# GaetanBenoitDev/metaMDBG

Measured on AMD Instinct MI355X. Metric: Gbp/s through minimizer+k-min-mer step; bit-exact k-min-mer table vs ref, higher is better.
Workload: dtype u64

## Files before the change

include/mdbg_hip.h:

```cpp
#ifndef MDBG_HIP_H
#define MDBG_HIP_H

#include <stddef.h>
#include <stdint.h>

#ifdef __cplusplus
extern "C" {
#endif

#define MDBG_OK        0
#define MDBG_EINVAL   -1
#define MDBG_ENODEV   -2
#define MDBG_ENOMEM   -3
#define MDBG_EHIP     -4
#define MDBG_ERANGE   -5
#define MDBG_EPEER    -6

typedef struct mdbg_ctx mdbg_ctx;
typedef struct mdbg_reads mdbg_reads;
typedef struct mdbg_minimizers mdbg_minimizers;
typedef struct mdbg_table mdbg_table;

int  mdbg_create(int device, mdbg_ctx **ctx);
void mdbg_destroy(mdbg_ctx *ctx);
// ... 76 lines not shown
                              mdbg_table **out);
int  mdbg_prev_from_records(mdbg_ctx *ctx, const uint8_t *records20, uint64_t n_records, mdbg_table **out);
int  mdbg_prev_overlay_unitigs(mdbg_ctx *ctx, mdbg_table *prev, const mdbg_minimizers *unitigs,
                               const uint32_t *abundance, uint32_t k_prev);
int  mdbg_kminmer_count_refined(mdbg_ctx *ctx, const mdbg_minimizers *reads, const mdbg_minimizers *unitigs,
                                uint32_t k, const mdbg_table *prev, mdbg_table **out);
int  mdbg_kminmer_index(mdbg_ctx *ctx, const mdbg_minimizers *reads, const mdbg_minimizers *unitigs,
                        uint32_t k, const mdbg_table *prev, mdbg_table **out);

int  mdbg_small_contigs(mdbg_ctx *ctx, const mdbg_minimizers *unitigs, uint32_t k, uint32_t k_prev, const mdbg_table *prev,
                        uint8_t *flags);

int  mdbg_table_info(const mdbg_table *t, uint32_t *k, uint64_t *n_records, uint64_t *n_solid, int *has_vectors);
int  mdbg_table_to_host(mdbg_ctx *ctx, const mdbg_table *t, uint8_t *records20, uint32_t *vectors);
int  mdbg_table_to_host_range(mdbg_ctx *ctx, const mdbg_table *t, uint64_t first, uint64_t count, uint8_t *records20, uint32_t *vectors);
int  mdbg_table_stats(const mdbg_table *t, uint64_t stats[4]);
int  mdbg_first_pass_info(const mdbg_ctx *ctx, uint64_t info[8]);
int  mdbg_first_pass_form(const mdbg_ctx *ctx, uint64_t form[4]);
int  mdbg_first_pass_slot_fall_backs(const mdbg_ctx *ctx, uint64_t *n);
const char *mdbg_step_kernel_name(uint32_t index);
int  mdbg_kernel_attributes(mdbg_ctx *ctx, const char *kernel, uint64_t attr[8]);
int  mdbg_scan_info(const mdbg_ctx *ctx, uint64_t info[8]);
int  mdbg_scan_confirm_info(const mdbg_ctx *ctx, uint64_t info[4]);
int  mdbg_table_checksum(mdbg_ctx *ctx, const mdbg_table *t, uint64_t sums[4]);
int  mdbg_table_lookup(mdbg_ctx *ctx, const mdbg_table *t, const uint64_t *hash_lo, const uint64_t *hash_hi,
                       uint64_t n, uint32_t *abundance);
int  mdbg_edge_index(mdbg_ctx *ctx, const mdbg_table *nodes, mdbg_table **edges, uint64_t *checksum);
int  mdbg_table_keys_to_host(mdbg_ctx *ctx, const mdbg_table *t, uint64_t *keys_lo_hi);
int  mdbg_unitig_edge_index(mdbg_ctx *ctx, const mdbg_minimizers *unitigs, uint32_t k, mdbg_table **edges, uint64_t *checksum);
void mdbg_table_free(mdbg_table *t);

typedef struct mdbg_spans mdbg_spans;
int  mdbg_kminmer_spans(mdbg_ctx *ctx, const mdbg_reads *reads, const mdbg_minimizers *mins,
                        uint32_t minimizer_size, int32_t hpc, uint32_t k, mdbg_spans **out);
int  mdbg_spans_info(const mdbg_spans *s, uint32_t *n_reads, uint64_t *n_minimizers, uint64_t *n_windows, uint32_t *k);
int  mdbg_spans_to_host(mdbg_ctx *ctx, const mdbg_spans *s, uint64_t *window_offsets,
                        uint32_t *min_start, uint32_t *min_end,
                        uint64_t *hash_lo, uint64_t *hash_hi, uint8_t *reversed,
                        uint32_t *pos_start, uint32_t *pos_end, uint32_t *seq_length_start, uint32_t *seq_length_end);
int  mdbg_spans_device_ptrs(const mdbg_spans *s, const uint64_t **d_window_offsets, const uint64_t **d_hash_lo, const uint64_t **d_hash_hi,
                            const uint32_t **d_pos_start, const uint32_t **d_pos_end);
void mdbg_spans_free(mdbg_spans *s);

typedef struct { uint64_t window; uint32_t part; uint32_t reserved; } mdbg_seq_request;
typedef struct { uint32_t read, start, length, reversed; } mdbg_seq_range;
enum { MDBG_SEQ_ENTIRE = 0, MDBG_SEQ_LEFT = 1, MDBG_SEQ_RIGHT = 2 };
// ... 85 lines not shown
```

metamdbg_amd/capi.py:

```python
from __future__ import annotations

import ctypes as C
import os

import numpy as np

_HERE = os.path.dirname(os.path.abspath(__file__))
LIB_PATH = os.environ.get("MDBG_LIB") or os.path.join(_HERE, "libmdbg_hip.so")

MDBG_READ_LOW_COMPLEXITY = 1
MDBG_READ_LOW_QUALITY = 2
RECORDS_PLAIN, RECORDS_INIT = 0, 1
SEQ_ENTIRE, SEQ_LEFT, SEQ_RIGHT = 0, 1, 2
SEQ_BITSET, SEQ_ASCII = 0, 1
SEQ_REQUEST = np.dtype([("window", "<u8"), ("part", "<u4"), ("reserved", "<u4")])
SEQ_RANGE = np.dtype([("read", "<u4"), ("start", "<u4"), ("length", "<u4"), ("reversed", "<u4")])


class MdbgError(RuntimeError):
    def __init__(self, code: int, msg: str):
        super().__init__(f"libmdbg_hip error {code}: {msg}")
        self.code = code


# ... 42 lines not shown
    "mdbg_minimizers_device_ptrs": (C.c_int, [_P, C.POINTER(_P), C.POINTER(_P)]),
    "mdbg_minimizers_free": (None, [_P]),
    "mdbg_minimizers_concat": (C.c_int, [_P, C.POINTER(_P), C.c_uint32, C.POINTER(_P)]),
    "mdbg_apply_density_threshold": (C.c_int, [_P, _P, C.c_float, C.POINTER(_P)]),
    "mdbg_purge_palindromes": (C.c_int, [_P, _P, C.c_uint32, C.c_uint32, C.POINTER(_P)]),
    "mdbg_repetitive_minimizers": (C.c_int, [_P, _P, _P, _u32p]),
    "mdbg_census_create": (C.c_int, [_P, C.POINTER(_P)]),
    "mdbg_census_add": (C.c_int, [_P, _P, _P]),
    "mdbg_census_top": (C.c_int, [_P, _P, _P, _u32p]),
    "mdbg_census_free": (None, [_P]),
    "mdbg_kminmer_count_first": (C.c_int, [_P, _P, C.c_uint32, C.c_uint32, C.POINTER(_P)]),
    "mdbg_prev_from_records": (C.c_int, [_P, _P, C.c_uint64, C.POINTER(_P)]),
    "mdbg_prev_overlay_unitigs": (C.c_int, [_P, _P, _P, _P, C.c_uint32]),
    "mdbg_kminmer_count_refined": (C.c_int, [_P, _P, _P, C.c_uint32, _P, C.POINTER(_P)]),
    "mdbg_kminmer_index": (C.c_int, [_P, _P, _P, C.c_uint32, _P, C.POINTER(_P)]),
    "mdbg_table_info": (C.c_int, [_P, _u32p, _u64p, _u64p, C.POINTER(C.c_int)]),
    "mdbg_table_to_host": (C.c_int, [_P, _P, _P, _P]),
    "mdbg_table_to_host_range": (C.c_int, [_P, _P, C.c_uint64, C.c_uint64, _P, _P]),
    "mdbg_table_checksum": (C.c_int, [_P, _P, _u64p]),
    "mdbg_table_stats": (C.c_int, [_P, _u64p]),
    "mdbg_first_pass_info": (C.c_int, [_P, _u64p]),
    "mdbg_scan_info": (C.c_int, [_P, _u64p]),
    "mdbg_scan_confirm_info": (C.c_int, [_P, _u64p]),
    "mdbg_first_pass_form": (C.c_int, [_P, _u64p]),
    "mdbg_first_pass_slot_fall_backs": (C.c_int, [_P, _u64p]),
    "mdbg_step_kernel_name": (C.c_char_p, [C.c_uint32]),
    "mdbg_kernel_attributes": (C.c_int, [_P, C.c_char_p, _u64p]),
    "mdbg_stream_spin": (C.c_int, [_P, C.c_uint32]),
    "mdbg_minimizers_slice": (C.c_int, [_P, _P, C.c_uint32, C.c_uint32, C.POINTER(C.c_void_p)]),
    "mdbg_shard_exchange_local": (C.c_int, [_P, C.POINTER(C.c_void_p), C.c_uint32, C.POINTER(C.c_void_p), _u64p, C.POINTER(C.c_void_p)]),
    "mdbg_device_clock_khz": (C.c_int, [_P, C.POINTER(C.c_int)]),
    "mdbg_table_lookup": (C.c_int, [_P, _P, _P, _P, C.c_uint64, _P]),
    "mdbg_edge_index": (C.c_int, [_P, _P, C.POINTER(_P), _u64p]),
    "mdbg_unitig_edge_index": (C.c_int, [_P, _P, C.c_uint32, C.POINTER(_P), _u64p]),
    "mdbg_small_contigs": (C.c_int, [_P, _P, C.c_uint32, C.c_uint32, _P, _P]),
    "mdbg_table_keys_to_host": (C.c_int, [_P, _P, _P]),
    "mdbg_table_free": (None, [_P]),
    "mdbg_kminmer_spans": (C.c_int, [_P, _P, _P, C.c_uint32, C.c_int32, C.c_uint32, C.POINTER(_P)]),
    "mdbg_spans_info": (C.c_int, [_P, _u32p, _u64p, _u64p, _u32p]),
    "mdbg_spans_to_host": (C.c_int, [_P, _P, _P, _P, _P, _P, _P, _P, _P, _P, _P, _P]),
    "mdbg_spans_device_ptrs": (C.c_int, [_P, C.POINTER(_P), C.POINTER(_P), C.POINTER(_P), C.POINTER(_P), C.POINTER(_P)]),
    "mdbg_spans_free": (None, [_P]),
    "mdbg_spans_extract": (C.c_int, [_P, _P, _P, _P, C.c_uint64, C.c_int, C.POINTER(_P)]),
    "mdbg_reads_extract_ranges": (C.c_int, [_P, _P, _P, C.c_uint64, C.c_int, C.POINTER(_P)]),
    "mdbg_sequences_info": (C.c_int, [_P, _u64p, _u64p, _u64p, C.POINTER(C.c_int)]),
    "mdbg_sequences_to_host": (C.c_int, [_P, _P, _P, _P, _P]),
# ... 124 lines not shown
            names.append(name.decode())
            i += 1
        return names

    def kernel_attributes(self, kernel: str) -> dict:
        a = (C.c_uint64 * 8)()
        self.check(lib().mdbg_kernel_attributes(self.h, kernel.encode(), a))
        names = ("registers", "static_lds", "max_threads", "threads", "role", "scratch")
        return {k: int(v) for k, v in zip(names, a)}

    def scan_info(self) -> dict:
        a = (C.c_uint64 * 8)()
        self.check(lib().mdbg_scan_info(self.h, a))
        names = ("prefiltered_launches", "block_launches", "bitmaps_built", "bitmap_bits_set", "bitmap_log2_bits", "prefilter_waves",
                 "last_prefiltered", "reads_segmented")
        return {k: int(v) for k, v in zip(names, a)}

    def scan_confirm_info(self) -> dict:
        a = (C.c_uint64 * 4)()
        self.check(lib().mdbg_scan_confirm_info(self.h, a))
        names = ("tables_built", "table_buckets", "table_overflowed", "last_by_table")
        return {k: int(v) for k, v in zip(names, a)}

    def timing(self, on: bool) -> None:
        self.check(lib().mdbg_timing_enable(self.h, int(on)))

    def timing_reset(self) -> None:
        self.check(lib().mdbg_timing_reset(self.h))

    def timing_get(self, kernel: str) -> tuple[float, int]:
        ms, n = C.c_double(), C.c_uint64()
        self.check(lib().mdbg_timing_get(self.h, kernel.encode(), C.byref(ms), C.byref(n)))
        return ms.value, n.value

    def reads_from_ascii(self, seqs: list[bytes], quals: list[bytes] | None = None) -> "Reads":
        offs = np.zeros(len(seqs) + 1, dtype=np.uint64)
        np.cumsum([len(s) for s in seqs], out=offs[1:])
        bases = b"".join(seqs)
        q = b"".join(quals) if quals is not None else None
        h = C.c_void_p()
        self.check(lib().mdbg_reads_from_ascii(self.h, bases, q, _ptr(offs), len(seqs), C.byref(h)))
        return Reads(self, h)

    def reads_from_packed(self, words: np.ndarray, word_off: np.ndarray, lens: np.ndarray, quals: list[bytes] | None = None) -> "Reads":
        words = np.ascontiguousarray(words, dtype=np.uint64)
        word_off = np.ascontiguousarray(word_off, dtype=np.uint64)
# ... 639 lines not shown
```

metamdbg_amd/csrc/common.hpp:

```cpp
#pragma once
#include <ctime>
#include <cstdio>
#include <cstdlib>

#include <hip/hip_runtime.h>

#include <cstdarg>
#include <cstdint>
#include <cstdio>
#include <cstring>
#include <map>
#include <memory>
#include <mutex>
#include <new>
#include <stdexcept>
#include <string>
#include <unordered_map>
#include <utility>
#include <vector>

#include "../../include/mdbg_hip.h"
#include "segments_dev.hpp"

namespace mdbg {
// ... 104 lines not shown
    unsigned table_blocks_per_cu = 1024;
    unsigned scan_reads_per_wave = 0;
    uint32_t scan_wave_priority = 0;
    int test_exchange_fail_phase = 0;
    bool test_corrupt_replies = false;
    uint32_t scan_cand_slack = 0;
    uint32_t scan_guard_slack = 0;
    uint32_t scan_prefilter = 1;
    uint32_t scan_prefilter_log2_bits = 0;
    uint32_t *prefilter_bits = nullptr;
    bool prefilter_valid = false;
    uint64_t prefilter_threshold = 0;
    uint32_t prefilter_log2 = 0, prefilter_set = 0;
    uint32_t scan_confirm_table = 0;
    uint32_t scan_confirm_table_log2_buckets = 0;
    uint32_t *confirm_table = nullptr;
    bool confirm_valid = false;
    uint64_t confirm_threshold = 0;
    uint32_t confirm_log2 = 0;
    uint64_t scan_confirm_info[4] = {0};
    uint32_t scan_segments = 1;
    uint32_t scan_segment_bases = mdbg::SEG_DEFAULT_BASES;
    uint64_t scan_info[8] = {0};
    double key_ratio_hint[4] = {0.0625, 0.0625, 0.0625, 0.0625};
    bool key_ratio_known[4] = {false, false, false, false};
    int first_pass_mode = 0;
    uint64_t part_auto_min = 1ull << 17;
    uint32_t part_bits = 0;
    uint32_t part_lds_slots = 0;
    uint64_t part_max_records = 0;
    uint32_t part_tile = 0;
    uint32_t part_threads = 0;
    uint64_t part_form[4] = {0};
    uint64_t part_fell_back = 0;
    uint32_t part_slot_list = 1;
    uint32_t scan_lds_pad = 0;
    uint32_t scan_lds_reserve = 0;
    size_t lds_per_cu = 0;
    uint32_t index_table_form = 1;
    uint32_t refined_form = 1;
    uint32_t scan_quality_beside = 1;
    uint32_t keep_index_table = 1;
    double index_last_miss_fraction = -1.0;
    uint32_t index_tuning = INDEX_TUNING_DEFAULT;
    uint64_t part_info[8] = {0};
    std::shared_ptr<mdbg::DevPool> pool;
// ... 185 lines not shown
```

metamdbg_amd/csrc/context.hip:

```cpp
#include "common.hpp"

#include <algorithm>
#include <cstdlib>

namespace mdbg {

thread_local std::string g_last_error;

int set_error(mdbg_ctx *ctx, int code, const char *fmt, ...) {
    char buf[1024];
    va_list ap;
    va_start(ap, fmt);
    vsnprintf(buf, sizeof(buf), fmt, ap);
    va_end(ap);
    if (ctx) ctx->err = buf; else g_last_error = buf;
    return code;
}

static void fold_timers(mdbg_ctx *ctx) {
    if (ctx->launches.empty()) return;
    (void)hipStreamSynchronize(ctx->stream);
    if (ctx->side_stream) (void)hipStreamSynchronize(ctx->side_stream);
    for (auto &t : ctx->launches) {
        float ms = 0;
// ... 20 lines not shown
    if (e != hipSuccess || count == 0)
        return set_error(nullptr, MDBG_ENODEV, "mdbg_create: no HIP device (%s); this library has no CPU path",
                         e != hipSuccess ? hipGetErrorString(e) : "device count is 0");
    if (device < 0 || device >= count)
        return set_error(nullptr, MDBG_EINVAL, "mdbg_create: device %d out of range (%d devices)", device, count);
    hipDeviceProp_t prop;
    if ((e = hipGetDeviceProperties(&prop, device)) != hipSuccess)
        return set_error(nullptr, MDBG_EHIP, "hipGetDeviceProperties: %s", hipGetErrorString(e));
    if (strncmp(prop.gcnArchName, "gfx950", 6) != 0)
        return set_error(nullptr, MDBG_ENODEV, "mdbg_create: device %d is %s; kernels are built for gfx950 only",
                         device, prop.gcnArchName);
    if ((e = hipSetDevice(device)) != hipSuccess)
        return set_error(nullptr, MDBG_EHIP, "hipSetDevice: %s", hipGetErrorString(e));
    mdbg_ctx *ctx = new mdbg_ctx();
    ctx->device = device;
    ctx->arch = prop.gcnArchName;
    ctx->n_cu = prop.multiProcessorCount;
    if (const char *e = getenv("MDBG_TABLE_BLOCKS_PER_CU")) if (atoi(e) > 0) ctx->table_blocks_per_cu = (unsigned)atoi(e);
    if (const char *e = getenv("MDBG_SCAN_WAVE_PRIORITY")) ctx->scan_wave_priority = (uint32_t)std::max(0, std::min(3, atoi(e)));
    if (const char *e = getenv("MDBG_SCAN_READS_PER_WAVE")) if (atoi(e) > 0) ctx->scan_reads_per_wave = (unsigned)atoi(e);
    if (const char *e = getenv("MDBG_SCAN_LDS_RESERVE")) ctx->scan_lds_reserve = (uint32_t)std::max(0, std::min(131072, atoi(e)));
    if (const char *e = getenv("MDBG_SCAN_PREFILTER")) ctx->scan_prefilter = atoi(e) != 0;
    if (const char *e = getenv("MDBG_SCAN_CONFIRM_TABLE")) ctx->scan_confirm_table = atoi(e) != 0;
    if (const char *e = getenv("MDBG_SCAN_SEGMENTS")) ctx->scan_segments = atoi(e) == 0 ? 0u : (atoi(e) == 2 ? 2u : 1u);
    if (const char *e = getenv("MDBG_SCAN_LDS_PAD")) ctx->scan_lds_pad = (uint32_t)std::max(0, std::min(32768, atoi(e)));
    if (const char *e = getenv("MDBG_PARTITION_TILE")) ctx->part_tile = atoi(e) == 2048 ? 2048u : 0u;
    if (const char *e = getenv("MDBG_PARTITION_THREADS")) ctx->part_threads = atoi(e) == 256 ? 256u : (atoi(e) == 512 ? 512u : 0u);
    if (const char *e = getenv("MDBG_PARTITION_SLOT_LIST")) ctx->part_slot_list = atoi(e) != 0;
    if (const char *e = getenv("MDBG_FIRST_PASS_MODE")) ctx->first_pass_mode = std::max(0, std::min(2, atoi(e)));
    ctx->hbm_bytes = prop.totalGlobalMem;
    ctx->lds_per_cu = prop.maxSharedMemoryPerMultiProcessor;
    ctx->clock_khz = prop.clockRate;
    if ((e = hipStreamCreateWithFlags(&ctx->stream, hipStreamNonBlocking)) != hipSuccess ||
        (e = hipStreamCreateWithFlags(&ctx->side_stream, hipStreamNonBlocking)) != hipSuccess) {
        if (ctx->stream) (void)hipStreamDestroy(ctx->stream);
        delete ctx;
        return set_error(nullptr, MDBG_EHIP, "hipStreamCreate: %s", hipGetErrorString(e));
    }
    ctx->pool = std::make_shared<DevPool>();
    ctx->pool->device = device;
    if (ctx->hbm_bytes) ctx->pool->cache_limit = std::max<size_t>(ctx->pool->cache_limit, (size_t)((double)ctx->hbm_bytes * 0.55));
    *out = ctx;
    return MDBG_OK;
} MDBG_API_CATCH((mdbg_ctx *)nullptr)

extern "C" void mdbg_destroy(mdbg_ctx *ctx) {
    if (!ctx) return;
    (void)hipSetDevice(ctx->device);
    fold_timers(ctx);
    (void)hipStreamSynchronize(ctx->stream);
    if (ctx->pool) ctx->pool->close();
    if (ctx->scan_stream) { (void)hipStreamSynchronize(ctx->scan_stream); (void)hipStreamDestroy(ctx->scan_stream); }
    if (ctx->upload_stream) { (void)hipStreamSynchronize(ctx->upload_stream); (void)hipStreamDestroy(ctx->upload_stream); }
    if (ctx->side_stream) { (void)hipStreamSynchronize(ctx->side_stream); (void)hipStreamDestroy(ctx->side_stream); }
    if (ctx->pinned) (void)hipHostFree(ctx->pinned);
    if (ctx->prefilter_bits) { std::lock_guard<std::mutex> g(hip_mem_mutex()); (void)hipFree(ctx->prefilter_bits); }
    if (ctx->confirm_table) { std::lock_guard<std::mutex> g(hip_mem_mutex()); (void)hipFree(ctx->confirm_table); }
    if (ctx->stream) (void)hipStreamDestroy(ctx->stream);
    delete ctx;
}

extern "C" const char *mdbg_last_error(const mdbg_ctx *ctx) {
    return ctx ? ctx->err.c_str() : g_last_error.c_str();
}

extern "C" int mdbg_synchronize(mdbg_ctx *ctx) try {
    if (!ctx) return MDBG_EINVAL;
    MDBG_HIP_CHECK(ctx, hipStreamSynchronize(ctx->stream));
    return MDBG_OK;
} MDBG_API_CATCH(ctx)

__global__ void spin_kernel(long long ticks) {
    const long long t0 = wall_clock64();
    while (wall_clock64() - t0 < ticks) __builtin_amdgcn_s_sleep(8);
}

extern "C" int mdbg_stream_spin(mdbg_ctx *ctx, uint32_t microseconds) try {
    if (!ctx) return MDBG_EINVAL;
    MDBG_HIP_CHECK(ctx, hipSetDevice(ctx->device));
    int khz = 0;
// ... 34 lines not shown
extern "C" int mdbg_set_option(mdbg_ctx *ctx, const char *name, int64_t value) {
    if (!ctx || !name) return set_error(ctx, MDBG_EINVAL, "mdbg_set_option: null argument");
    const std::string n(name);
    if (n == "pool_cache_percent") {
        const int64_t pc = value > 0 ? std::min<int64_t>(value, 95) : 55;
        std::lock_guard<std::mutex> g(ctx->pool->mu);
        ctx->pool->cache_limit = std::max<size_t>((size_t)96 << 30, (size_t)((double)ctx->hbm_bytes * (double)pc / 100.0));
        return MDBG_OK;
    }
    if (n == "pool_trim") {
        MDBG_HIP_CHECK(ctx, hipSetDevice(ctx->device));
        MDBG_HIP_CHECK(ctx, hipStreamSynchronize(ctx->stream));
        ctx->pool->trim();
        return MDBG_OK;
    }
    if (n == "table_cu_count") return set_table_cu_count(ctx, value > 0 ? (unsigned)std::min<int64_t>(value, 4096) : 0u);
    if (n == "table_grid_blocks") { ctx->table_grid_blocks = value > 0 ? (unsigned)std::min<int64_t>(value, 1 << 20) : 0u; return MDBG_OK; }
    if (n == "table_blocks_per_cu") { ctx->table_blocks_per_cu = value > 0 ? (unsigned)std::min<int64_t>(value, 1024) : 1024u; return MDBG_OK; }
    if (n == "scan_wave_priority") { ctx->scan_wave_priority = (uint32_t)std::max<int64_t>(0, std::min<int64_t>(3, value)); return MDBG_OK; }
    if (n == "scan_candidate_slack") { ctx->scan_cand_slack = value > 0 ? (uint32_t)std::min<int64_t>(value, 1 << 24) : 0u; return MDBG_OK; }
    if (n == "scan_guard_slack") { ctx->scan_guard_slack = value > 0 ? (uint32_t)std::min<int64_t>(value, 0xFFFFFFFFll - 68) : 0u; return MDBG_OK; }
    if (n == "scan_prefilter") { ctx->scan_prefilter = value != 0; return MDBG_OK; }
    if (n == "scan_confirm_table") { ctx->scan_confirm_table = value != 0; return MDBG_OK; }
    if (n == "scan_confirm_table_log2_buckets") {
        if (value != 0 && (value < 10 || value > 16)) return set_error(ctx, MDBG_EINVAL, "scan_confirm_table_log2_buckets: 0 (the kernel's own) or 10 .. 16");
        ctx->scan_confirm_table_log2_buckets = (uint32_t)value; return MDBG_OK;
    }
    if (n == "scan_segments") {
        if (value > 2) return set_error(ctx, MDBG_EINVAL, "scan_segments: 0 (never), 1 (automatic, the default; negative too) or 2 (every eligible read)");
        ctx->scan_segments = value < 0 ? 1u : (uint32_t)value; return MDBG_OK;
    }
    if (n == "scan_segment_bases") {
        if (value > 0 && (value % 2048 != 0 || value > (1 << 30))) return set_error(ctx, MDBG_EINVAL, "scan_segment_bases: a multiple of 2048 (<= 0: the default, 16384)");
        ctx->scan_segment_bases = value <= 0 ? SEG_DEFAULT_BASES : (uint32_t)value; return MDBG_OK;
    }
    if (n == "scan_prefilter_log2_bits") {
        if (value != 0 && (value < 10 || value > 19)) return set_error(ctx, MDBG_EINVAL, "scan_prefilter_log2_bits: 0 (the kernel's own) or 10 .. 19");
        ctx->scan_prefilter_log2_bits = (uint32_t)value; return MDBG_OK;
    }
    if (n == "scan_reads_per_wave") { ctx->scan_reads_per_wave = value > 0 ? (unsigned)std::min<int64_t>(value, 1 << 20) : 0u; return MDBG_OK; }
    if (n == "first_pass_mode") { ctx->first_pass_mode = (int)std::max<int64_t>(0, std::min<int64_t>(2, value)); return MDBG_OK; }
    if (n == "partition_auto_min") { ctx->part_auto_min = value > 0 ? (uint64_t)value : (1ull << 17); return MDBG_OK; }
    if (n == "partition_bits") { ctx->part_bits = (uint32_t)std::max<int64_t>(0, std::min<int64_t>(24, value)); return MDBG_OK; }
    if (n == "partition_lds_slots") {
        if (value != 0 && value != 256 && value != 1024 && value != 2048) return set_error(ctx, MDBG_EINVAL, "partition_lds_slots: 0, 256, 1024 or 2048");
        ctx->part_lds_slots = (uint32_t)value; return MDBG_OK;
// ... 72 lines not shown
```

metamdbg_amd/csrc/partition.hip:

```cpp
#include "common.hpp"
#include "kminmer_dev.hpp"
#include "partition_plan.hpp"

#include <algorithm>
#include <cmath>
#include <vector>

namespace mdbg {

#ifndef MDBG_PART_NT
#define MDBG_PART_NT 512
#endif
#ifndef MDBG_PART_E
#define MDBG_PART_E 8
#endif
constexpr uint32_t PART_NT = MDBG_PART_NT;
constexpr uint32_t PART_E = MDBG_PART_E;
constexpr uint32_t PART_TILE = PART_NT * PART_E;
constexpr uint32_t PART_MAXW = 256;
constexpr uint32_t PART_NT_SMALL = 256;
constexpr uint32_t PART_E_SMALL = 4;
constexpr uint32_t PART_TILE_SMALL = PART_NT_SMALL * PART_E_SMALL;
static_assert(PART_NT_SMALL >= PART_MAXW && PART_NT >= PART_MAXW, "the scatter scans a tile's histogram with one thread per way");
constexpr uint32_t PART_MAX_K = 32;
// ... 565 lines not shown
    for (uint64_t i = tid; i < n; i += BC_NT) {
        const uint32_t row = in.rep[s0 + i];
        const uint32_t s = lds_find<C>(t, in.lo[s0 + i], in.hi[s0 + i]);
        reply[row] = (uint64_t)t.cnt[s] | (t.rep[s] == row ? (1ull << 63) : 0ull);
    }
}

struct RecBufs {
    DevBuf<unsigned long long> lo, hi;
    DevBuf<uint32_t> rep;
    uint64_t cap = 0;
    int ensure(mdbg_ctx *ctx, uint64_t n) {
        if (n <= cap) return MDBG_OK;
        MDBG_TRY(lo.alloc(ctx, n)); MDBG_TRY(hi.alloc(ctx, n)); MDBG_TRY(rep.alloc(ctx, n));
        cap = n;
        return MDBG_OK;
    }
    RecView view() { return RecView{lo.p, hi.p, rep.p}; }
};

struct SplitForm { uint32_t threads, tile; };

static SplitForm split_form(const mdbg_ctx *ctx) {
    if (ctx->part_threads == PART_NT_SMALL) return SplitForm{PART_NT_SMALL, PART_TILE_SMALL};
    return SplitForm{PART_NT, ctx->part_tile == 2048 ? PART_TILE / 2 : PART_TILE};
}

static void launch_split_hist(mdbg_ctx *ctx, bool from_mins, SplitForm f, unsigned grid, const SplitArgs &a, uint32_t *hist) {
    if (f.threads == PART_NT_SMALL && PART_NT_SMALL != PART_NT) {
        if (from_mins) hipLaunchKernelGGL((split_hist_kernel<true, PART_NT_SMALL>), dim3(grid), dim3(PART_NT_SMALL), 0, ctx->stream, a, hist);
        else hipLaunchKernelGGL((split_hist_kernel<false, PART_NT_SMALL>), dim3(grid), dim3(PART_NT_SMALL), 0, ctx->stream, a, hist);
    } else {
        if (from_mins) hipLaunchKernelGGL((split_hist_kernel<true, PART_NT>), dim3(grid), dim3(PART_NT), 0, ctx->stream, a, hist);
        else hipLaunchKernelGGL((split_hist_kernel<false, PART_NT>), dim3(grid), dim3(PART_NT), 0, ctx->stream, a, hist);
    }
    ctx->part_form[0] = f.threads; ctx->part_form[1] = f.tile;
}

static void launch_split_scatter(mdbg_ctx *ctx, bool from_mins, SplitForm f, unsigned grid, const SplitArgs &a, const uint64_t *place, RecView out) {
    if (f.tile == PART_TILE_SMALL && f.threads == PART_NT_SMALL) {
        if (from_mins) hipLaunchKernelGGL((split_scatter_kernel<true, PART_E_SMALL, PART_NT_SMALL>), dim3(grid), dim3(PART_NT_SMALL), 0, ctx->stream, a, place, out);
        else hipLaunchKernelGGL((split_scatter_kernel<false, PART_E_SMALL, PART_NT_SMALL>), dim3(grid), dim3(PART_NT_SMALL), 0, ctx->stream, a, place, out);
    } else if (f.tile != PART_TILE) {
        if (from_mins) hipLaunchKernelGGL((split_scatter_kernel<true, PART_E / 2, PART_NT>), dim3(grid), dim3(PART_NT), 0, ctx->stream, a, place, out);
        else hipLaunchKernelGGL((split_scatter_kernel<false, PART_E / 2, PART_NT>), dim3(grid), dim3(PART_NT), 0, ctx->stream, a, place, out);
    } else {
        if (from_mins) hipLaunchKernelGGL((split_scatter_kernel<true, PART_E, PART_NT>), dim3(grid), dim3(PART_NT), 0, ctx->stream, a, place, out);
// ... 550 lines not shown
```

metamdbg_amd/csrc/scan.hip:

```cpp
#include "common.hpp"
#include "complexity_dev.hpp"
#include "murmur.hpp"
#include "objects.hpp"
#include "prefilter.hpp"
#include "scan_plan.hpp"
#include "segments_dev.hpp"

#include <fcntl.h>
#include <sys/file.h>
#include <sys/stat.h>
#include <unistd.h>

#include <algorithm>
#include <cerrno>
#include <cmath>
#include <cstdlib>
#include <memory>
#include <mutex>
#include <string>
#include <thread>
#include <type_traits>

namespace mdbg {

// ... 31 lines not shown
    uint8_t *out_mqual;
    int inline_minq;
    uint32_t *out_count;
    uint8_t *out_flags;
    unsigned long long *cursor;
    uint32_t n_regions;
    uint64_t out_capacity;
    uint64_t *out_begin;
    uint32_t *over_list, *suspect_list;
    uint32_t *list_counters;
    const uint8_t *skip;
    uint32_t cand_slack;
    uint32_t guard_slack;
    uint32_t wave_priority;
    const uint32_t *pf_bits;
    uint32_t pf_shift;
    uint32_t pf_chunk;
    const uint4 *pf_table;
    uint32_t pf_table_shift;
    uint32_t pf_len_split;
    const SegView *views;
    unsigned long long *view_cx;
    uint32_t seg_tiles;
};

__device__ __forceinline__ uint64_t compress_pairs(uint64_t x, uint64_t d) {
    uint64_t xm = x & (d | (d << 1));
    uint32_t xl = (uint32_t)xm, xh = (uint32_t)(xm >> 32);
    uint32_t dl = (uint32_t)d, dh = (uint32_t)(d >> 32);
    uint32_t lo = 0, hi = 0;
    unsigned n = 0;
#pragma unroll
    for (int i = 0; i < 16; i++) {
        lo |= ((xl >> (2 * i)) & 3u) << n;
        n += (dl >> (2 * i) & 1u) << 1;
    }
    const unsigned nlo = n;
    n = 0;
#pragma unroll
    for (int i = 0; i < 16; i++) {
        hi |= ((xh >> (2 * i)) & 3u) << n;
        n += (dh >> (2 * i) & 1u) << 1;
    }
    return (uint64_t)lo | ((uint64_t)hi << nlo);
}

// ... 631 lines not shown
    uint16_t *hist_o = lds_hist_o + ((QUAL && HPC) ? wv * HIST_TILES * 64 : 0);
    uint32_t *hist_c = lds_hist_c[(QUAL && HPC) ? wv : 0];
    const unsigned K = a.K;
    const uint32_t kmask = (K >= 16) ? 0xFFFFFFFFu : ((1u << (2 * K)) - 1u);
    const uint32_t comp_mask = 0xAAAAAAAAu & kmask;
    const unsigned top_shift = 2u * K - 2u;
    const uint64_t threshold = a.threshold;
    const uint64_t cand_limit64 = (threshold >> 32) + 3ull + (uint64_t)a.cand_slack;
    const uint32_t cand_limit = cand_limit64 > 0xFFFFFFFFull ? 0xFFFFFFFFu : (uint32_t)cand_limit64;
    const uint64_t guard_limit64 = 68ull + (uint64_t)a.guard_slack;
    const uint32_t guard_limit = guard_limit64 > 0xFFFFFFFFull ? 0xFFFFFFFFu : (uint32_t)guard_limit64;
    const bool unguarded = HPC && K == 15u && a.guard_slack == 0u;

    const uint32_t wave_global = blockIdx.x * Geo::WAVES + wv;
    const uint32_t n_waves = gridDim.x * Geo::WAVES;
    uint16_t *pf_list = PF ? pf_list_all + wv * PF_LIST_CAP : nullptr;
    uint32_t *pf_surv = PF ? pf_surv_all + wv * 64u : nullptr;
    const uint32_t pf_shift = a.pf_shift;
    const uint4 *const pf_table = PF ? a.pf_table : nullptr;
    const uint32_t pf_table_shift = a.pf_table_shift;
    constexpr uint32_t NO_READ = 0xFFFFFFFFu;
    const uint64_t chunk0 = (uint64_t)blockIdx.x * a.pf_chunk;
    const uint32_t chunk_n = PF ? (chunk0 >= a.n_reads ? 0u : (uint32_t)(a.n_reads - chunk0 < a.pf_chunk ? a.n_reads - chunk0 : a.pf_chunk)) : 0u;
    auto take_read = [&]() -> uint32_t {
        uint32_t k = 0;
        if (lane == 0) k = atomicAdd(pf_next, 1u);
        k = (uint32_t)__builtin_amdgcn_readfirstlane((int)k);
        return k < chunk_n ? (uint32_t)chunk0 + k : NO_READ;
    };
    for (uint32_t r = PF ? take_read() : wave_global; PF ? r != NO_READ : r < a.n_reads; r = PF ? take_read() : r + n_waves) {
        if constexpr (PF && !SEG) { if (a.pf_len_split && a.len[r] >= a.pf_len_split) continue; }
        if (!SEG && a.skip && a.skip[r]) {
            if (a.cursor && lane == 0) { a.out_begin[r] = 0; a.out_count[r] = 0; a.out_flags[r] = 0; }
            continue;
        }
        SegView view{};
        if constexpr (SEG) {
            view = a.views[r];
            if (view.flags & SEG_DEAD) {
                if (lane == 0) { a.out_begin[r] = 0; a.out_count[r] = 0; a.out_flags[r] = 0; a.view_cx[r] = 0ull; }
                continue;
            }
        }
        const uint32_t rd = SEG ? view.read : r;
        const bool seg_inner = SEG && !(view.flags & SEG_FIRST);
        const uint32_t L = SEG ? view.raw_len : a.len[r];
        const uint64_t w_base = a.word_off[rd] + (SEG ? (uint64_t)view.tile0 * TILE_WORDS : 0ull);
// ... 481 lines not shown
            materialise();
            release_ring(((fill + 15u) & ~15u) + 16u);
        }

        if (APPROX && !PF) {
            const uint32_t n_staged = outgrown ? n_staged_at_outgrowth : nout;
            for (uint32_t i = lane; i < ((n_staged + 63u) & ~63u); i += 64) {
                const uint64_t fb = __ballot(i < n_staged && !(kmer_hash32(stage[i].x) < threshold));
                if (fb) { n_false += (uint32_t)__popcll(fb); lost = true; }
            }
        }
        if (((QUAL && HPC) || (APPROX && !PF)) && __ballot(lost) != 0ull) outgrown = true;
        uint8_t flags = 0;
        if constexpr (SEG) {
            const uint64_t cx_view = a.apply_filters ? cx_total + wave_sum_u32(cx_acc) : 0ull;
            if (lane == 0) a.view_cx[r] = cx_view;
        } else if (a.apply_filters && L >= 66) {
            if (complexity_suspect(cx_total + wave_sum_u32(cx_acc), cx_nW)) flags |= READ_SUSPECT;
        }
        if (bump) {
            uint64_t start = 0;
            if (!outgrown && nout) {
                uint32_t lo = 0, hi = 0;
                const uint32_t region = wave_global & (a.n_regions - 1u);
                if (lane == 0) { const unsigned long long s0 = atomicAdd(a.cursor + region, (unsigned long long)nout); lo = (uint32_t)s0; hi = (uint32_t)(s0 >> 32); }
                start = ((uint64_t)(uint32_t)__builtin_amdgcn_readfirstlane((int)hi) << 32) | (uint32_t)__builtin_amdgcn_readfirstlane((int)lo);
                const bool fits = start + nout <= a.out_capacity;
                start += (uint64_t)region * a.out_capacity;
                if (fits) {
                    for (uint32_t i = lane; i < nout; i += 64) {
                        const uint2 e = stage[i];
                        a.out_min[start + i] = e.x; a.out_pos[start + i] = e.y >> 1; a.out_dir[start + i] = (uint8_t)(e.y & 1u);
                        if (QUAL) a.out_mqual[start + i] = stage_q[i];
                    }
                }
            }
            if (lane == 0) {
                a.out_begin[r] = start;
                a.out_count[r] = nout - n_false;
                a.out_flags[r] = flags;
                if (outgrown) a.over_list[atomicAdd(&a.list_counters[0], 1u)] = r;
                if (flags & READ_SUSPECT) a.suspect_list[atomicAdd(&a.list_counters[1], 1u)] = r;
            }
        } else {
            const uint32_t ns = nout - flushed;
            for (uint32_t i = lane; i < ns; i += 64) {
                const uint32_t idx = flushed + i;
// ... 503 lines not shown
        if (!(fast && ctx->scan_stream)) return MDBG_OK;
        MDBG_HIP_CHECK(ctx, hipEventCreateWithFlags(&ordered, hipEventDisableTiming));
        hipError_t e = hipEventRecord(ordered, ctx->stream);
        if (e == hipSuccess) e = hipStreamWaitEvent(ctx->scan_stream, ordered, 0);
        if (e != hipSuccess) { (void)hipEventDestroy(ordered); return set_error(ctx, MDBG_EHIP, "scan stream hand-over: %s", hipGetErrorString(e)); }
        on = ctx->scan_stream;
        return MDBG_OK;
    }
    int give_back(mdbg_ctx *ctx) {
        if (!ordered) return MDBG_OK;
        hipError_t e = hipEventRecord(ordered, on);
        if (e == hipSuccess) e = hipStreamWaitEvent(ctx->stream, ordered, 0);
        (void)hipEventDestroy(ordered);
        if (e != hipSuccess) return set_error(ctx, MDBG_EHIP, "scan stream hand-back: %s", hipGetErrorString(e));
        return MDBG_OK;
    }
};

static unsigned four_wave_lds_pad(const mdbg_ctx *ctx, ScanKernel fk) {
    const bool by_reserve = !ctx->scan_lds_pad && ctx->scan_lds_reserve;
    return scan_lds_padding(ctx->scan_lds_pad, ctx->scan_lds_reserve, ctx->lds_per_cu, by_reserve ? kernel_static_lds(reinterpret_cast<const void *>(fk)) : 0);
}

static int launch_scan(mdbg_ctx *ctx, ScanArgs &a, bool hpc, bool has_q, bool has_n, uint32_t n_items, uint32_t pf_len_limit = 0, bool pf_split = false,
                       uint64_t batch_bases = 0, bool seg = false) {
    a.n_reads = n_items;
    const ScanSwitches &sw = scan_switches();
    const bool fast = (!has_q || a.cursor) && !has_n && !a.subset && !sw.no_fast;
    const bool approx = fast && a.cursor && sw.approx_allowed && candidate_test_usable(a.threshold, a.cand_slack);
    if (seg && !approx) return set_error(ctx, MDBG_EINVAL, "scan: views are scanned by the candidate-hash kernels only");
    unsigned pf_waves = 0;
    MDBG_TRY(choose_prefilter(ctx, a, approx, hpc, has_q, pf_len_limit, &pf_waves));
    pf_split = pf_split && pf_waves;
    DevBuf<uint8_t> d_split;
    if (pf_split) {
        MDBG_TRY(split_long_reads(ctx, a, n_items, pf_len_limit, batch_bases, d_split, &pf_split));
        if (!pf_split) pf_waves = 0;
    }
    ScanStreamLoan loan;
    MDBG_TRY(loan.take(ctx, fast));
    if (fast) ctx->scan_info[6] = pf_waves ? 1 : 0;
    if (fast) ctx->scan_confirm_info[3] = 0;
    {
        LaunchTimer timer(ctx, "scan", loan.on);
        const uint8_t *const batch_skip = a.skip;
        if (pf_split) a.skip = d_split.p;
        if (fast && (!pf_waves || pf_split)) {
            ctx->scan_info[1]++;
            const ScanKernel fk = select_fast_kernel(hpc, has_q, approx, 0, seg);
            hipLaunchKernelGGL(fk, dim3(scan_blocks(n_items, FAST_WAVES, ctx->scan_reads_per_wave)), dim3(FAST_BLOCK), four_wave_lds_pad(ctx, fk), loan.on, a);
        } else if (!fast) {
            hipLaunchKernelGGL(select_general_kernel(hpc, has_q, has_n), dim3(scan_blocks(n_items, SCAN_WAVES, ctx->scan_reads_per_wave)), dim3(SCAN_BLOCK), 0, ctx->stream, a);
        }
        a.skip = batch_skip;
        if (pf_waves) {
            a.pf_bits = ctx->prefilter_bits;
            a.pf_shift = 32u - ctx->prefilter_log2;
            const bool by_table = ctx->scan_confirm_table && ctx->confirm_valid && ctx->confirm_threshold == a.threshold;
            a.pf_table = by_table ? reinterpret_cast<const uint4 *>(ctx->confirm_table) : nullptr;
            a.pf_table_shift = by_table ? 32u - ctx->confirm_log2 : 0u;
            ctx->scan_confirm_info[3] = by_table ? 1 : 0;
            const PrefilterGrid grid = prefilter_grid(n_items, pf_waves, ctx->scan_reads_per_wave, ctx->n_cu);
            a.pf_chunk = grid.chunk;
            a.pf_len_split = pf_split ? pf_len_limit : 0u;
            hipLaunchKernelGGL(select_fast_kernel(true, false, true, pf_waves, seg), dim3(grid.blocks), dim3(64u * pf_waves), 0, loan.on, a);
            ctx->scan_info[0]++; ctx->scan_info[5] = pf_waves;
        }
    }
    MDBG_TRY(loan.give_back(ctx));
    MDBG_HIP_CHECK(ctx, hipGetLastError());
    return MDBG_OK;
}

struct SegPlan : SegTotals {
    DevBuf<uint32_t> tiles_per_read, views_per_read, tile_runs, tile_excl;
    DevBuf<uint64_t> tile_off, view_off;
    DevBuf<SegView> views;
    DevBuf<uint8_t> skip, read_cut;
    DevBuf<unsigned long long> totals;
};

static int seg_prepass(mdbg_ctx *ctx, const mdbg_reads *reads, const uint8_t *masked, uint32_t G, uint32_t K, bool hpc, SegPlan &sp) {
    const uint32_t n = reads->n_reads;
    const uint64_t max_tiles = reads->n_bases / SEG_TILE_BASES + n, max_views = reads->n_bases / G + n;
    MDBG_TRY(sp.tiles_per_read.alloc(ctx, n)); MDBG_TRY(sp.views_per_read.alloc(ctx, n));
    MDBG_TRY(sp.tile_off.alloc(ctx, (size_t)n + 1)); MDBG_TRY(sp.view_off.alloc(ctx, (size_t)n + 1));
    MDBG_TRY(sp.tile_runs.alloc(ctx, hpc ? max_tiles : 1)); MDBG_TRY(sp.tile_excl.alloc(ctx, hpc ? max_tiles : 1));
    MDBG_TRY(sp.views.alloc(ctx, max_views)); MDBG_TRY(sp.skip.alloc(ctx, n)); MDBG_TRY(sp.read_cut.alloc(ctx, n)); MDBG_TRY(sp.totals.alloc(ctx, 8));
// ... 455 lines not shown
    e = hipMemcpyAsync(m->d_len.p, reads->d_len.p, (size_t)n * 4, hipMemcpyDeviceToDevice, ctx->stream);
    if (e != hipSuccess) return set_error(ctx, MDBG_EHIP, "len copy failed: %s", hipGetErrorString(e));
    MDBG_TRY(j.quality.start(ctx, reads, m.get(), j.has_q));

    const ScanSwitches &sw = scan_switches();
    const BlockRoute route = plan_block_route(n, reads->n_bases, reads->max_len, p->density, j.hpc, j.has_n, reads->d_masked.p != nullptr, j.has_n ? reads->n_masked : 0u,
                                              sw.bump_allowed, STAGE_CAP);
    SegPlan seg;
    if (segments_wanted(route, ctx->scan_segments, reads->max_len, ctx->scan_segment_bases, STAGE_CAP, sw.approx_allowed, density_threshold(p->density), ctx->scan_cand_slack))
        MDBG_TRY(seg_prepass(ctx, reads, route.route_masked ? reads->d_masked.p : nullptr, ctx->scan_segment_bases, p->minimizer_size, j.hpc, seg));
    bool done = false;
    if (route.block_path_but_length && (route.avg_fits_stage || seg.n_cut)) MDBG_TRY(j.scan_block_path(route, seg, &done));
    if (!done) MDBG_TRY(j.scan_general_path());
    *out = m.release();
    return MDBG_OK;
} MDBG_API_CATCH(ctx)

extern "C" int mdbg_scan_confirm_info(const mdbg_ctx *ctx, uint64_t info[4]) {
    if (!ctx || !info) return MDBG_EINVAL;
    for (int i = 0; i < 4; i++) info[i] = ctx->scan_confirm_info[i];
    return MDBG_OK;
}

extern "C" int mdbg_scan_info(const mdbg_ctx *ctx, uint64_t info[8]) {
    if (!ctx || !info) return MDBG_EINVAL;
    for (int i = 0; i < 8; i++) info[i] = ctx->scan_info[i];
    return MDBG_OK;
}

namespace mdbg {
const StepKernel *scan_step_kernels(uint32_t *n) {
    static const StepKernel k[] = {
        {"scan_prefiltered_16", reinterpret_cast<const void *>(scan_fast_kernel<true, false, true, 16>), 1024, 0},
    };
    *n = (uint32_t)(sizeof(k) / sizeof(k[0]));
    return k;
}
}
```

metamdbg_amd/csrc/scan_plan.hpp:

```cpp
#pragma once
#include <algorithm>
#include <cstddef>
#include <cstdint>
#include <vector>

namespace mdbg {

inline bool candidate_test_usable(uint64_t threshold, uint32_t cand_slack) { return (threshold >> 32) + 3ull + (uint64_t)cand_slack < 0xFFFFFFFFull; }

struct BlockRoute {
    bool route_masked, block_path_but_length, avg_fits_stage;
    double rows_per_base;
};
inline BlockRoute plan_block_route(uint32_t n, uint64_t n_bases, uint32_t max_len, float density, bool hpc, bool has_n, bool masked_listed, uint32_t n_masked,
                                   bool bump_allowed, int stage_cap) {
    BlockRoute r;
    r.route_masked = has_n && masked_listed && (uint64_t)n_masked * 8ull <= (uint64_t)n + 128ull;
    r.block_path_but_length = n && (!has_n || r.route_masked) && bump_allowed && density < 0.2f && max_len < (1u << 31);
    r.rows_per_base = (double)density * (hpc ? 0.8 : 1.0) * 1.4;
    r.avg_fits_stage = n && (double)n_bases / (double)n * r.rows_per_base + 24.0 < (double)stage_cap;
    return r;
}

inline bool segments_wanted(const BlockRoute &r, uint32_t scan_segments, uint32_t max_len, uint32_t seg_G, int stage_cap, bool approx_allowed, uint64_t threshold,
// ... 40 lines not shown
constexpr unsigned SCAN_READS_PER_WAVE = 2, PREFILTER_READS_PER_WAVE = 32, PREFILTER_MIN_GROUPS_PER_CU = 2;

inline unsigned prefilter_reads_per_wave(int n_cu, uint32_t n_items, unsigned waves) {
    unsigned per_wave = PREFILTER_READS_PER_WAVE;
    const uint64_t want = (uint64_t)PREFILTER_MIN_GROUPS_PER_CU * (uint64_t)std::max(n_cu, 1);
    while (per_wave > SCAN_READS_PER_WAVE && (uint64_t)n_items / ((uint64_t)waves * per_wave) < want) per_wave /= 2;
    return per_wave;
}

inline unsigned scan_blocks(uint32_t n_items, int waves, uint32_t reads_per_wave_option) {
    const uint64_t per_wave = reads_per_wave_option ? reads_per_wave_option : SCAN_READS_PER_WAVE;
    uint64_t blocks = ((uint64_t)n_items + waves * per_wave - 1) / (waves * per_wave);
    if (blocks < 1) blocks = 1;
    if (blocks > 0x7FFFFFFFull) blocks = 0x7FFFFFFFull;
    return (unsigned)blocks;
}
struct PrefilterGrid { uint32_t chunk; unsigned blocks; };
inline PrefilterGrid prefilter_grid(uint32_t n_items, unsigned pf_waves, uint32_t reads_per_wave_option, int n_cu) {
    const uint64_t chunk = std::min<uint64_t>((uint64_t)pf_waves * (reads_per_wave_option ? reads_per_wave_option : prefilter_reads_per_wave(n_cu, n_items, pf_waves)), 1u << 24);
    const uint64_t blocks = std::min<uint64_t>(std::max<uint64_t>(1, ((uint64_t)n_items + chunk - 1) / chunk), 0x7FFFFFFFull);
    return PrefilterGrid{(uint32_t)chunk, (unsigned)blocks};
}

inline size_t lds_of_a_cu(size_t lds_per_cu) { return lds_per_cu ? lds_per_cu : 163840u; }
inline unsigned prefilter_wave_count(size_t lds_per_cu, size_t reserve, size_t lds16, size_t lds8) {
    const size_t total = lds_of_a_cu(lds_per_cu);
    const size_t room = total > reserve ? total - reserve : 0;
    return lds16 <= room ? 16u : lds8 <= room ? 8u : 0u;
}
inline unsigned scan_lds_padding(unsigned pad_option, size_t reserve, size_t lds_per_cu, size_t lds) {
    unsigned lds_pad = pad_option;
    if (lds_pad || !reserve || !lds) return lds_pad;
    const size_t total = lds_of_a_cu(lds_per_cu);
    size_t fit = total > reserve ? (total - reserve) / lds : 1;
    if (fit < 2) fit = 2;
    const size_t need = total / (fit + 1) + 1;
    if (need > lds) lds_pad = (unsigned)(((need - lds) + 255u) / 256u * 256u);
    const size_t most = (size_t)65536 > lds ? (size_t)65536 - lds : 0;
    if (lds_pad > most) lds_pad = (unsigned)(most / 256u * 256u);
    return lds_pad;
}

struct Placement {
    std::vector<uint32_t> list[2], cnt[2];
    std::vector<uint64_t> start[2];
    uint64_t rows;
// ... 20 lines not shown
```

Measured before the change: 1244.

## Make the prefiltered scan persistent with a global atomic read counter

The prefiltered scan kernel now launches one workgroup per CU by default, and each wave grabs runs of reads from a single device-wide atomic counter instead of working through a fixed per-block chunk. The output region is chosen from the run index rather than the wave index, and a small ring of device counters is allocated and zeroed before each launch. The partition kernel also switches to its small-thread form when it runs next to the persistent scan. The aim is better load balance over reads of uneven length and less launch-tail imbalance, at the cost of more atomic contention on one counter and an extra memset per launch.

New measurement: 1270, median of 6. +2.1%, better.

```diff
diff --git a/include/mdbg_hip.h b/include/mdbg_hip.h
--- a/include/mdbg_hip.h
+++ b/include/mdbg_hip.h
@@ -122,6 +122,7 @@
 int  mdbg_kernel_attributes(mdbg_ctx *ctx, const char *kernel, uint64_t attr[8]);
 int  mdbg_scan_info(const mdbg_ctx *ctx, uint64_t info[8]);
 int  mdbg_scan_confirm_info(const mdbg_ctx *ctx, uint64_t info[4]);
+int  mdbg_scan_persistent_info(const mdbg_ctx *ctx, uint64_t info[4]);
 int  mdbg_table_checksum(mdbg_ctx *ctx, const mdbg_table *t, uint64_t sums[4]);
 int  mdbg_table_lookup(mdbg_ctx *ctx, const mdbg_table *t, const uint64_t *hash_lo, const uint64_t *hash_hi,
                        uint64_t n, uint32_t *abundance);
diff --git a/metamdbg_amd/capi.py b/metamdbg_amd/capi.py
--- a/metamdbg_amd/capi.py
+++ b/metamdbg_amd/capi.py
@@ -88,6 +88,7 @@
     "mdbg_first_pass_info": (C.c_int, [_P, _u64p]),
     "mdbg_scan_info": (C.c_int, [_P, _u64p]),
     "mdbg_scan_confirm_info": (C.c_int, [_P, _u64p]),
+    "mdbg_scan_persistent_info": (C.c_int, [_P, _u64p]),
     "mdbg_first_pass_form": (C.c_int, [_P, _u64p]),
     "mdbg_first_pass_slot_fall_backs": (C.c_int, [_P, _u64p]),
     "mdbg_step_kernel_name": (C.c_char_p, [C.c_uint32]),
@@ -258,6 +259,11 @@
         names = ("tables_built", "table_buckets", "table_overflowed", "last_by_table")
         return {k: int(v) for k, v in zip(names, a)}
 
+    def scan_persistent_info(self) -> dict:
+        a = (C.c_uint64 * 4)()
+        self.check(lib().mdbg_scan_persistent_info(self.h, a))
+        return {"form": "persistent" if a[0] else "chunked", "workgroups": int(a[1]), "grab_reads": int(a[2]), "persistent_launches": int(a[3])}
+
     def timing(self, on: bool) -> None:
         self.check(lib().mdbg_timing_enable(self.h, int(on)))
 
diff --git a/metamdbg_amd/csrc/common.hpp b/metamdbg_amd/csrc/common.hpp
--- a/metamdbg_amd/csrc/common.hpp
+++ b/metamdbg_amd/csrc/common.hpp
@@ -150,6 +150,13 @@
     uint32_t scan_segments = 1;
     uint32_t scan_segment_bases = mdbg::SEG_DEFAULT_BASES;
     uint64_t scan_info[8] = {0};
+    uint32_t scan_persistent = 1;
+    uint32_t scan_grab_reads = 0;
+    uint32_t scan_persistent_blocks = 0;
+    static constexpr uint32_t SCAN_COUNTER_SLOTS = 16;
+    unsigned long long *scan_counters = nullptr;
+    uint32_t scan_counter_next = 0;
+    uint64_t scan_persistent_info[4] = {0};
     double key_ratio_hint[4] = {0.0625, 0.0625, 0.0625, 0.0625};
     bool key_ratio_known[4] = {false, false, false, false};
     int first_pass_mode = 0;
diff --git a/metamdbg_amd/csrc/context.hip b/metamdbg_amd/csrc/context.hip
--- a/metamdbg_amd/csrc/context.hip
+++ b/metamdbg_amd/csrc/context.hip
@@ -66,6 +66,8 @@
     if (const char *e = getenv("MDBG_SCAN_LDS_RESERVE")) ctx->scan_lds_reserve = (uint32_t)std::max(0, std::min(131072, atoi(e)));
     if (const char *e = getenv("MDBG_SCAN_PREFILTER")) ctx->scan_prefilter = atoi(e) != 0;
     if (const char *e = getenv("MDBG_SCAN_CONFIRM_TABLE")) ctx->scan_confirm_table = atoi(e) != 0;
+    if (const char *e = getenv("MDBG_SCAN_PERSISTENT")) ctx->scan_persistent = atoi(e) != 0;
+    if (const char *e = getenv("MDBG_SCAN_GRAB_READS")) ctx->scan_grab_reads = (uint32_t)std::max(0, std::min(1 << 16, atoi(e)));
     if (const char *e = getenv("MDBG_SCAN_SEGMENTS")) ctx->scan_segments = atoi(e) == 0 ? 0u : (atoi(e) == 2 ? 2u : 1u);
     if (const char *e = getenv("MDBG_SCAN_LDS_PAD")) ctx->scan_lds_pad = (uint32_t)std::max(0, std::min(32768, atoi(e)));
     if (const char *e = getenv("MDBG_PARTITION_TILE")) ctx->part_tile = atoi(e) == 2048 ? 2048u : 0u;
@@ -100,6 +102,7 @@
     if (ctx->pinned) (void)hipHostFree(ctx->pinned);
     if (ctx->prefilter_bits) { std::lock_guard<std::mutex> g(hip_mem_mutex()); (void)hipFree(ctx->prefilter_bits); }
     if (ctx->confirm_table) { std::lock_guard<std::mutex> g(hip_mem_mutex()); (void)hipFree(ctx->confirm_table); }
+    if (ctx->scan_counters) { std::lock_guard<std::mutex> g(hip_mem_mutex()); (void)hipFree(ctx->scan_counters); }
     if (ctx->stream) (void)hipStreamDestroy(ctx->stream);
     delete ctx;
 }
@@ -180,6 +183,9 @@
     if (n == "scan_guard_slack") { ctx->scan_guard_slack = value > 0 ? (uint32_t)std::min<int64_t>(value, 0xFFFFFFFFll - 68) : 0u; return MDBG_OK; }
     if (n == "scan_prefilter") { ctx->scan_prefilter = value != 0; return MDBG_OK; }
     if (n == "scan_confirm_table") { ctx->scan_confirm_table = value != 0; return MDBG_OK; }
+    if (n == "scan_persistent") { ctx->scan_persistent = value != 0; return MDBG_OK; }
+    if (n == "scan_grab_reads") { ctx->scan_grab_reads = (uint32_t)std::max<int64_t>(0, std::min<int64_t>(1 << 16, value)); return MDBG_OK; }
+    if (n == "scan_persistent_blocks") { ctx->scan_persistent_blocks = (uint32_t)std::max<int64_t>(0, std::min<int64_t>(1 << 20, value)); return MDBG_OK; }
     if (n == "scan_confirm_table_log2_buckets") {
         if (value != 0 && (value < 10 || value > 16)) return set_error(ctx, MDBG_EINVAL, "scan_confirm_table_log2_buckets: 0 (the kernel's own) or 10 .. 16");
         ctx->scan_confirm_table_log2_buckets = (uint32_t)value; return MDBG_OK;
diff --git a/metamdbg_amd/csrc/partition.hip b/metamdbg_amd/csrc/partition.hip
--- a/metamdbg_amd/csrc/partition.hip
+++ b/metamdbg_amd/csrc/partition.hip
@@ -611,7 +611,8 @@
 struct SplitForm { uint32_t threads, tile; };
 
 static SplitForm split_form(const mdbg_ctx *ctx) {
-    if (ctx->part_threads == PART_NT_SMALL) return SplitForm{PART_NT_SMALL, PART_TILE_SMALL};
+    const bool beside_persistent_scan = ctx->part_threads == 0 && ctx->scan_lds_reserve && ctx->scan_persistent && ctx->scan_info[6] && ctx->scan_persistent_info[0];
+    if (ctx->part_threads == PART_NT_SMALL || beside_persistent_scan) return SplitForm{PART_NT_SMALL, PART_TILE_SMALL};
     return SplitForm{PART_NT, ctx->part_tile == 2048 ? PART_TILE / 2 : PART_TILE};
 }
 
diff --git a/metamdbg_amd/csrc/scan.hip b/metamdbg_amd/csrc/scan.hip
--- a/metamdbg_amd/csrc/scan.hip
+++ b/metamdbg_amd/csrc/scan.hip
@@ -77,6 +77,8 @@
     const SegView *views;
     unsigned long long *view_cx;
     uint32_t seg_tiles;
+    unsigned long long *pf_counter;
+    uint32_t pf_grab;
 };
 
 __device__ __forceinline__ uint64_t compress_pairs(uint64_t x, uint64_t d) {
@@ -754,7 +756,24 @@
     constexpr uint32_t NO_READ = 0xFFFFFFFFu;
     const uint64_t chunk0 = (uint64_t)blockIdx.x * a.pf_chunk;
     const uint32_t chunk_n = PF ? (chunk0 >= a.n_reads ? 0u : (uint32_t)(a.n_reads - chunk0 < a.pf_chunk ? a.n_reads - chunk0 : a.pf_chunk)) : 0u;
+    unsigned long long *const pf_counter = PF ? a.pf_counter : nullptr;
+    uint32_t run_next = 0, run_end = 0, run_region = 0;
     auto take_read = [&]() -> uint32_t {
+        if (pf_counter) {
+            if (run_next == run_end) {
+                uint32_t lo = 0, hi = 0;
+                if (lane == 0) {
+                    const unsigned long long s0 = __hip_atomic_fetch_add(pf_counter, (unsigned long long)a.pf_grab, __ATOMIC_RELAXED, __HIP_MEMORY_SCOPE_AGENT);
+                    lo = (uint32_t)s0; hi = (uint32_t)(s0 >> 32);
+                }
+                lo = (uint32_t)__builtin_amdgcn_readfirstlane((int)lo); hi = (uint32_t)__builtin_amdgcn_readfirstlane((int)hi);
+                if (hi || lo >= a.n_reads) return NO_READ;
+                run_next = lo;
+                run_end = a.n_reads - lo < a.pf_grab ? a.n_reads : lo + a.pf_grab;
+                run_region = (lo / a.pf_grab) & (a.n_regions - 1u);
+            }
+            return run_next++;
+        }
         uint32_t k = 0;
         if (lane == 0) k = atomicAdd(pf_next, 1u);
         k = (uint32_t)__builtin_amdgcn_readfirstlane((int)k);
@@ -1282,7 +1301,7 @@
             uint64_t start = 0;
             if (!outgrown && nout) {
                 uint32_t lo = 0, hi = 0;
-                const uint32_t region = wave_global & (a.n_regions - 1u);
+                const uint32_t region = pf_counter ? run_region : wave_global & (a.n_regions - 1u);
                 if (lane == 0) { const unsigned long long s0 = atomicAdd(a.cursor + region, (unsigned long long)nout); lo = (uint32_t)s0; hi = (uint32_t)(s0 >> 32); }
                 start = ((uint64_t)(uint32_t)__builtin_amdgcn_readfirstlane((int)hi) << 32) | (uint32_t)__builtin_amdgcn_readfirstlane((int)lo);
                 const bool fits = start + nout <= a.out_capacity;
@@ -1832,9 +1851,22 @@
     return scan_lds_padding(ctx->scan_lds_pad, ctx->scan_lds_reserve, ctx->lds_per_cu, by_reserve ? kernel_static_lds(reinterpret_cast<const void *>(fk)) : 0);
 }
 
+static int scan_counter_take(mdbg_ctx *ctx, hipStream_t on, unsigned long long **counter) {
+    if (!ctx->scan_counters) {
+        std::lock_guard<std::mutex> g(hip_mem_mutex());
+        hipError_t e = hipMalloc((void **)&ctx->scan_counters, mdbg_ctx::SCAN_COUNTER_SLOTS * sizeof(unsigned long long));
+        if (e != hipSuccess) { ctx->scan_counters = nullptr; return set_error(ctx, MDBG_ENOMEM, "hipMalloc of the scan's read counters: %s", hipGetErrorString(e)); }
+    }
+    *counter = ctx->scan_counters + ctx->scan_counter_next;
+    ctx->scan_counter_next = (ctx->scan_counter_next + 1u) % mdbg_ctx::SCAN_COUNTER_SLOTS;
+    MDBG_HIP_CHECK(ctx, hipMemsetAsync(*counter, 0, sizeof(unsigned long long), on));
+    return MDBG_OK;
+}
+
 static int launch_scan(mdbg_ctx *ctx, ScanArgs &a, bool hpc, bool has_q, bool has_n, uint32_t n_items, uint32_t pf_len_limit = 0, bool pf_split = false,
                        uint64_t batch_bases = 0, bool seg = false) {
     a.n_reads = n_items;
+    a.pf_counter = nullptr; a.pf_grab = 0;
     const ScanSwitches &sw = scan_switches();
     const bool fast = (!has_q || a.cursor) && !has_n && !a.subset && !sw.no_fast;
     const bool approx = fast && a.cursor && sw.approx_allowed && candidate_test_usable(a.threshold, a.cand_slack);
@@ -1870,10 +1902,23 @@
             a.pf_table = by_table ? reinterpret_cast<const uint4 *>(ctx->confirm_table) : nullptr;
             a.pf_table_shift = by_table ? 32u - ctx->confirm_log2 : 0u;
             ctx->scan_confirm_info[3] = by_table ? 1 : 0;
-            const PrefilterGrid grid = prefilter_grid(n_items, pf_waves, ctx->scan_reads_per_wave, ctx->n_cu);
-            a.pf_chunk = grid.chunk;
             a.pf_len_split = pf_split ? pf_len_limit : 0u;
-            hipLaunchKernelGGL(select_fast_kernel(true, false, true, pf_waves, seg), dim3(grid.blocks), dim3(64u * pf_waves), 0, loan.on, a);
+            if (persistent_taken(ctx->scan_persistent, ctx->scan_reads_per_wave)) {
+                unsigned long long *counter = nullptr;
+                MDBG_TRY(scan_counter_take(ctx, loan.on, &counter));
+                a.pf_counter = counter;
+                a.pf_grab = persistent_grab(ctx->scan_grab_reads);
+                a.pf_chunk = 0;
+                const unsigned blocks = persistent_grid(n_items, pf_waves, a.pf_grab, ctx->n_cu, ctx->scan_persistent_blocks);
+                hipLaunchKernelGGL(select_fast_kernel(true, false, true, pf_waves, seg), dim3(blocks), dim3(64u * pf_waves), 0, loan.on, a);
+                ctx->scan_persistent_info[0] = 1; ctx->scan_persistent_info[1] = blocks; ctx->scan_persistent_info[2] = a.pf_grab; ctx->scan_persistent_info[3]++;
+            } else {
+                const PrefilterGrid grid = prefilter_grid(n_items, pf_waves, ctx->scan_reads_per_wave, ctx->n_cu);
+                a.pf_chunk = grid.chunk;
+                a.pf_counter = nullptr; a.pf_grab = 0;
+                hipLaunchKernelGGL(select_fast_kernel(true, false, true, pf_waves, seg), dim3(grid.blocks), dim3(64u * pf_waves), 0, loan.on, a);
+                ctx->scan_persistent_info[0] = 0; ctx->scan_persistent_info[1] = grid.blocks; ctx->scan_persistent_info[2] = 0;
+            }
             ctx->scan_info[0]++; ctx->scan_info[5] = pf_waves;
         }
     }
@@ -2375,6 +2420,12 @@
     return MDBG_OK;
 }
 
+extern "C" int mdbg_scan_persistent_info(const mdbg_ctx *ctx, uint64_t info[4]) {
+    if (!ctx || !info) return MDBG_EINVAL;
+    for (int i = 0; i < 4; i++) info[i] = ctx->scan_persistent_info[i];
+    return MDBG_OK;
+}
+
 extern "C" int mdbg_scan_info(const mdbg_ctx *ctx, uint64_t info[8]) {
     if (!ctx || !info) return MDBG_EINVAL;
     for (int i = 0; i < 8; i++) info[i] = ctx->scan_info[i];
diff --git a/metamdbg_amd/csrc/scan_plan.hpp b/metamdbg_amd/csrc/scan_plan.hpp
--- a/metamdbg_amd/csrc/scan_plan.hpp
+++ b/metamdbg_amd/csrc/scan_plan.hpp
@@ -86,6 +86,20 @@
     return PrefilterGrid{(uint32_t)chunk, (unsigned)blocks};
 }
 
+constexpr unsigned PERSISTENT_GRAB_READS = 4, PERSISTENT_GRAB_MAX = 1u << 16;
+inline unsigned persistent_grab(uint32_t grab_option) { return grab_option ? std::min<uint32_t>(grab_option, PERSISTENT_GRAB_MAX) : PERSISTENT_GRAB_READS; }
+inline bool persistent_taken(uint32_t persistent_option, uint32_t reads_per_wave_option) { return persistent_option && !reads_per_wave_option; }
+inline unsigned persistent_grid(uint32_t n_items, unsigned waves, unsigned grab, int n_cu, uint32_t blocks_cap) {
+    const uint64_t per_group = (uint64_t)waves * grab;
+    uint64_t blocks = std::min<uint64_t>(((uint64_t)n_items + per_group - 1) / per_group, (uint64_t)std::max(n_cu, 1));
+    if (blocks_cap) blocks = std::min<uint64_t>(blocks, blocks_cap);
+    return (unsigned)std::max<uint64_t>(blocks, 1);
+}
+inline uint32_t persistent_run_end(uint64_t start, unsigned grab, uint32_t n_items) {
+    return start >= n_items ? (uint32_t)n_items : (uint32_t)std::min<uint64_t>(start + grab, n_items);
+}
+inline uint32_t persistent_region(uint32_t item, unsigned grab, uint32_t n_regions) { return (item / grab) & (n_regions - 1u); }
+
 inline size_t lds_of_a_cu(size_t lds_per_cu) { return lds_per_cu ? lds_per_cu : 163840u; }
 inline unsigned prefilter_wave_count(size_t lds_per_cu, size_t reserve, size_t lds16, size_t lds8) {
     const size_t total = lds_of_a_cu(lds_per_cu);
```
